# TechPizzaDev/VorbisPizza

Measured on AMD Instinct MI355X. Metric: decoded PCM Msamples/s (batched stereo N=2048), higher is better.
Workload: dtype f32; 1 GPU; north_star: batched stereo 44.1 kHz N=2048 IMDCT + window + overlap-add to PCM through the fused kernel (Mdct.Reverse + OverlapBuffers + StoreContiguous, Mdct.cs:15-19 + StreamDecoder.cs:764-791, 594-638): 65536 all-long frames x 2 ch per GPU (BASELINE configs[1]'s batch taken all the way to PCM), spectra N(0, 2^-8) device-resident, planar float32 PCM out, 8 B per sample; frames_per_gpu=65536, channels=2, block_size=2048, device_state=steady: 200 untimed steps of the workload in front of the W warm-up steps

## Files before the change

vorbispizza_amd/csrc/steady_stereo.hip:

```cpp
#include "imdct_core.hpp"
#include "steady_map.hpp"
#include "synth_common.hpp"
#include "synth_desc.hpp"
#include "vpz_internal.hpp"

namespace vpz {

constexpr int kSteadyWaves = 4;
constexpr int kSteadyThreads = 64 * kSteadyWaves;

__global__ __launch_bounds__(kSteadyThreads, 2) void steady_stereo_kernel(SynthArgs a)
{
    __shared__ float2 s_scr[kSteadyWaves][2][kWaveScratchFloat2];
    __shared__ int s_done[kSteadyWaves];

    const int lane = threadIdx.x & 63;
    const int wave = __builtin_amdgcn_readfirstlane(threadIdx.x >> 6);
    const int run_idx = (int)blockIdx.x * kSteadyWaves + wave;
    const bool active = run_idx < a.n_runs;
    RunDesc run = a.runs[active ? run_idx : 0];
    float2 rtw[8], rtwAB[8], rtwBC[8];
    float w_lo[8], w_hi[8];
    {
        const VPZ_GLOBAL float2 *tw = (const VPZ_GLOBAL float2 *)a.tw_long;
        const VPZ_GLOBAL float *sl = (const VPZ_GLOBAL float *)a.slope1;
#pragma unroll
        for (int m = 0; m < 8; ++m) {
            rtw[m] = tw[kFastTwOffset + lane + 64 * m];
            rtwAB[m] = tw[kFastTwABOffset + 64 * m + lane];
            rtwBC[m] = tw[kFastTwBCOffset + 8 * (lane & 7) + m];
            const int k = steady::cur_index(lane, m);
            w_lo[m] = sl[steady::sample_lo(k)];
            w_hi[m] = sl[steady::sample_hi(k)];
        }
    }
    if (threadIdx.x < kSteadyWaves) s_done[threadIdx.x] = 0;
    __syncthreads();
    if (!active) return;

    float2 *scrL = s_scr[wave][0], *scrR = s_scr[wave][1];
    const int n_staged = run.count + (run.pre_kind == kPreRecompute ? 1 : 0);
    const bool defer = run.pre_kind == kPreNeighbour && wave > 0 && run.count > 0;
    const bool first_emits = run.pre_kind == kPreState;
    const VPZ_GLOBAL float2 *src = (const VPZ_GLOBAL float2 *)(a.spec + run.spec_base);
    const VPZ_GLOBAL float2 *idle = (const VPZ_GLOBAL float2 *)a.inv_db;
    float *row_l, *row_r;
    {
        float *ob = a.out + (a.stream_out_off ? a.stream_out_off[run.stream] : 0) + run.out_base;
        const uint64_t p = reinterpret_cast<uint64_t>(ob);
        const uint32_t lo = __builtin_amdgcn_readfirstlane((uint32_t)p), hi = __builtin_amdgcn_readfirstlane((uint32_t)(p >> 32));
        row_l = reinterpret_cast<float *>(((uint64_t)hi << 32) | lo);
        row_r = row_l + a.channel_stride;
    }
    const bool clip_on = a.clip != 0;
    float clip_peak = 0.0f;

    float tL[8], tR[8];
#pragma unroll
    for (int q = 0; q < 8; ++q) tL[q] = tR[q] = 0.0f;
    if (run.pre_kind == kPreState) {
        const VPZ_GLOBAL float *st = (const VPZ_GLOBAL float *)(a.state_h + (size_t)run.state_slot * a.state_slot_floats + (size_t)run.stream * 2 * 1024);
#pragma unroll
        for (int q = 0; q < 8; ++q) {
            tL[q] = st[steady::tail_index(lane, q)];
            tR[q] = st[1024 + steady::tail_index(lane, q)];
        }
    }
    float parkL[8], parkR[8];
#pragma unroll
    for (int q = 0; q < 8; ++q) parkL[q] = parkR[q] = 0.0f;

    auto prefetch = [&](const VPZ_GLOBAL float2 *s2, bool valid, float2 (&va)[8], float2 (&vb)[8]) {
        int l = lane;
        asm volatile("" : "+v"(l));
        const VPZ_GLOBAL float2 *p = valid ? s2 : idle;
        const int base = valid ? l : 0, step = valid ? 64 : 0, rofs = valid ? 512 : 0;
#pragma unroll
        for (int m = 0; m < 8; ++m) {
            va[m] = p[base + step * m];
            vb[m] = p[base + step * m + rofs];
        }
    };
    auto emit = [&](const float (&curL)[8], const float (&curR)[8], const float (&pL)[8], const float (&pR)[8], float *out_l, float *out_r) {
        float loL[8], hiL[8], loR[8], hiR[8];
#pragma unroll
        for (int q = 0; q < 8; ++q) {
            loL[q] = ola(-curL[q], w_lo[q], pL[q], w_hi[q]);
            hiL[q] = ola(curL[q], w_hi[q], pL[q], w_lo[q]);
            loR[q] = ola(-curR[q], w_lo[q], pR[q], w_hi[q]);
            hiR[q] = ola(curR[q], w_hi[q], pR[q], w_lo[q]);
        }
        if (clip_on) {
#pragma unroll
            for (int q = 0; q < 8; q += 2) {
                clip_group(loL[q], hiL[q], loL[q + 1], hiL[q + 1], clip_peak);
                clip_group(loR[q], hiR[q], loR[q + 1], hiR[q + 1], clip_peak);
            }
        }
        int lf = lane;
        asm volatile("" : "+v"(lf));
#pragma unroll
        for (int q = 0; q < 8; ++q) {
            const float gotL = lane_mirror64(q < 4 ? hiL[7 - q] : loL[7 - q], lf);
            const float gotR = lane_mirror64(q < 4 ? hiR[7 - q] : loR[7 - q], lf);
            const int at = q < 4 ? 512 + 2 * (lf + 64 * q) : 2 * (lf + 64 * q) - 512;
            vpz_f2v vl = {q < 4 ? hiL[q] : loL[q], gotL}, vr = {q < 4 ? hiR[q] : loR[q], gotR};
            __builtin_nontemporal_store(vl, (VPZ_GLOBAL vpz_f2v *)reinterpret_cast<vpz_f2v *>(out_l + at));
            __builtin_nontemporal_store(vr, (VPZ_GLOBAL vpz_f2v *)reinterpret_cast<vpz_f2v *>(out_r + at));
        }
    };

    float2 va[8], vb[8];
    prefetch(src, n_staged > 0, va, vb);
#pragma unroll
    for (int m = 0; m < 8; ++m) asm volatile("" ::"v"(va[m].x), "v"(va[m].y), "v"(vb[m].x), "v"(vb[m].y));

    float *out_l = row_l + (defer ? 1024 : 0), *out_r = row_r + (defer ? 1024 : 0);
#ifdef VPZ_STAMPS
    unsigned long long t_acc[12] = {0, 0, 0, 0, 0, 0, 0, 0, 0, 0, 0, 0};
    unsigned long long t_last = __builtin_amdgcn_s_memtime();
#endif
    const int iters = n_staged;
    for (int it = 0; it < iters; ++it) {
        float2 na[8], nb[8];
        src += 1024;
        prefetch(src, it + 1 < iters, na, nb);
        VPZ_STAMP(0);
        int ln = lane;
        asm volatile("" : "+v"(ln));
        float reL[8], nimL[8], reR[8], nimR[8];
        imdct2048_wave_x2_spectrum(va, vb, scrL, scrR, rtw, rtwAB, rtwBC, ln, reL, nimL, reR, nimR);
        VPZ_STAMP(3);
#pragma unroll
        for (int m = 0; m < 8; ++m) asm volatile("" ::"v"(na[m].x), "v"(na[m].y), "v"(nb[m].x), "v"(nb[m].y));
        VPZ_STAMP(4);
        float curL[8], curR[8];
// ... 41 lines not shown
        float *pubL = reinterpret_cast<float *>(scrL), *pubR = reinterpret_cast<float *>(scrR);
#pragma unroll
        for (int q = 0; q < 8; ++q) {
            pubL[64 * q + lane] = tL[q];
            pubR[64 * q + lane] = tR[q];
        }
        __builtin_amdgcn_fence(__ATOMIC_RELEASE, "workgroup");
        if (lane == 0) __hip_atomic_store(&s_done[wave], 1, __ATOMIC_RELAXED, __HIP_MEMORY_SCOPE_WORKGROUP);
    }
    if (defer) {
        int spins = 0;
        while (__hip_atomic_load(&s_done[wave - 1], __ATOMIC_RELAXED, __HIP_MEMORY_SCOPE_WORKGROUP) == 0 && ++spins < (1 << 23))
            __builtin_amdgcn_s_sleep(4);
        __builtin_amdgcn_fence(__ATOMIC_ACQUIRE, "workgroup");
        const float *nbL = reinterpret_cast<const float *>(s_scr[wave - 1][0]), *nbR = reinterpret_cast<const float *>(s_scr[wave - 1][1]);
        float pL[8], pR[8];
#pragma unroll
        for (int q = 0; q < 8; ++q) {
            pL[q] = nbL[64 * q + lane];
            pR[q] = nbR[64 * q + lane];
        }
        emit(parkL, parkR, pL, pR, row_l, row_r);
    }
    if (run.flags & kRunSaveState) {
        VPZ_GLOBAL float *st = (VPZ_GLOBAL float *)(a.state_h + (size_t)(run.state_slot ^ 1) * a.state_slot_floats + (size_t)run.stream * 2 * 1024);
#pragma unroll
        for (int q = 0; q < 8; ++q) {
            st[steady::tail_index(lane, q)] = tL[q];
            st[1024 + steady::tail_index(lane, q)] = tR[q];
        }
    }
    if (clip_on && __any(clip_peak > 0.99999994f) && lane == 0) atomicMax(&a.clipped[run.stream], run.clip_epoch);
}

hipError_t launch_steady_stereo(const SynthArgs &args, hipStream_t stream)
{
    if (args.n_runs <= 0) return hipSuccess;
    if (args.channels != 2 || args.size0 != 256 || args.size1 != 2048 || args.interleaved || args.s16 || args.spec_i16 || args.ccount != nullptr)
        return hipErrorInvalidValue;
    const int grid = (args.n_runs + kSteadyWaves - 1) / kSteadyWaves;
    hipLaunchKernelGGL(steady_stereo_kernel, dim3(grid), dim3(kSteadyThreads), 0, stream, args);
    return hipGetLastError();
}

}
```

vorbispizza_amd/csrc/synth_plan.hip:

```cpp
#include <cstdio>
#include <cstdlib>
#include <cstring>

#include "synth_plan.hpp"

namespace vpz {

constexpr int kCutSkewPermille = 25;

namespace {

constexpr int64_t kNone = INT64_MAX;


struct Prev {
    bool has_prev, prev_long;
    int prev_end, prev_stop;
};
inline Prev prev_of_state(const StreamState &S) { return Prev{S.has_prev, S.prev_long, S.prev_end, S.prev_stop}; }
inline Prev prev_of(const Decoder &D, const vpz_packet *packets, int64_t p)
{
    if (p > 0 && packets[p - 1].stream == packets[p].stream) {
        const vpz_packet &pp = packets[p - 1];
        const PacketInfo &ppi = D.packet_info[pp.flags & 7];
// ... 709 lines not shown
        for (int g = s_lo; g < s_hi; ++g) {
            const int cnt = segs[g].cnt, base = (int)W.s_base[segs[g].stream] + segs[g].off;
            if (c.reuse) (void)code_segment<false>(P, c, segs[g]);
            int64_t before = 0, run_units = 0;
            for (int f0 = 0; f0 < cnt; before += run_units) {
                const int len = c.batches ? run_length(c, W.cut_code.data() + base, f0, cnt, target_at(P, c, g, before, c.target_units), run_units)
                                          : std::min(c.R + (c.skew_frames ? ((int64_t)base + f0 < c.heavy_frames ? 1 : -1) : 0), cnt - f0);
                const RunDesc r = make_run(P, segs[g], f0, len);
                if (c.parties > 1) mine.push_back(r);
                else if (P.n_runs < P.runs_cap) P.runs[P.n_runs++] = r;
                else { P.host_failed = true; return; }
                f0 += len;
            }
        }
    });
    if (c.parties == 1 || P.host_failed) return;
    for (const std::vector<RunDesc> &v : cut) {
        if (P.n_runs + v.size() > P.runs_cap) { P.host_failed = true; return; }
        memcpy(P.runs + P.n_runs, v.data(), v.size() * sizeof(RunDesc));
        P.n_runs += v.size();
    }
}

void chain_runs(SynthPlan &P)
{
    const Decoder &D = P.D;
    const vpz_packet *packets = P.packets;
    RunDesc *runs = P.runs;
    const size_t n_runs = P.n_runs;
    P.n_chained = 0;
    if (!P.use_dual || !P.compact || D.size1 != 2048 || D.no_chain) return;
    const size_t waves = (size_t)P.dual_waves;
    auto chain_range = [&](size_t lo, size_t hi) -> int64_t {
        int64_t n = 0;
        for (size_t i = std::max<size_t>(lo, 1); i < hi; ++i) {
            RunDesc &r = runs[i];
            const RunDesc &pr = runs[i - 1];
            if (i % waves == 0 || r.pre_kind != kPreRecompute || r.stream != pr.stream || pr.count <= 0 ||
                r.first != pr.first + pr.count || !(r.flags & kRunCompact) || r.count <= 0)
                continue;
            const int64_t q = r.first;
            if (q <= 0 || packets[q - 1].stream != r.stream) continue;
            const uint8_t cf = P.cflags[q], pcf = P.cflags[q - 1];
            if ((cf & (7u | kCfSkip)) != 7u || (pcf & (1u | 4u | kCfSkip)) != 5u) continue;
            if (r.count == 1 && (r.flags & kRunLastTrimmed)) continue;
            r.pre_kind = kPreNeighbour;
            stage_from(P, r, q);
            ++n;
        }
        return n;
    };
    const bool want_inline = P.cut_R > 0 && P.cut_R + 1 <= 16;
    P.run_inline = want_inline ? arena_alloc<uint8_t>(*P.A, 32 * n_runs + 32) : nullptr;
    auto inline_range = [&](size_t lo, size_t hi) {
        for (size_t i = lo; want_inline && i < hi; ++i) {
            const RunDesc &r = runs[i];
            uint8_t *dst = P.run_inline + 32 * i;
            memset(dst, 0, 32);
            if (!(r.flags & kRunCompact)) continue;
            const int64_t q = (int64_t)r.first + (r.pre_kind == kPreRecompute ? -1 : 0);
            const int n = std::min(16, r.count + (r.pre_kind == kPreRecompute ? 1 : 0));
            for (int j = 0; j < n; ++j) {
                dst[j] = P.cflags[q + j];
                dst[16 + j] = P.cmap[q + j];
            }
        }
    };
    P.chain_threads = 1;
    if (P.pool && P.pool->parties() > 1 && n_runs >= 1024) {
        const int n_threads = P.chain_threads = P.pool->parties();
        std::vector<int64_t> part((size_t)n_threads, 0);
        P.host_failed |= !P.pool->run([&](int party) {
            const size_t lo = n_runs * (size_t)party / n_threads, hi = n_runs * (size_t)(party + 1) / n_threads;
            part[(size_t)party] = chain_range(lo, hi);
            inline_range(lo, hi);
        });
        for (int64_t v : part) P.n_chained += v;
    } else {
        P.n_chained = chain_range(0, n_runs);
        inline_range(0, n_runs);
    }
}

bool all_steady(const SynthPlan &P, const Cut &c)
{
    const Decoder &D = P.D;
    if (!P.use_dual || D.pairs || !P.compact || c.batches || D.no_steady || D.channels != 2 || D.size0 != 256 || D.size1 != 2048) return false;
    if (!P.facts.all_steady_flags || P.facts.any_floor || P.facts.any_short || P.facts.ilv_seen || !D.mismatch_packets.empty()) return false;
    for (int s = 0; s < D.n_streams; ++s) {
        if (D.plan.s_cnt[s] <= 0) continue;
        const StreamState &S = D.states[s];
        if (S.has_prev && !(S.prev_long && S.prev_end == 1024 && S.prev_stop == 2048)) return false;
        if (D.plan.trim_out_count[s] >= 0) return false;
    }
    return true;
}

}

bool SynthPlan::dual_usable() const
{
    if (!D.dual_ok || (facts.any_floor0 && !D.f0_fused) || (facts.ilv_seen && facts.planar_seen)) return false;
    const bool wide = facts.ilv_seen && !D.pairs;
// ... 38 lines not shown
                  W.cut_hint_R > 0;
        if (c.batches && W.cut_code.size() < (size_t)total_frames) W.cut_code.resize((size_t)total_frames);
        if (c.batches) W.s_units.assign((size_t)n_segs, 0);
        c.total_units = (c.batches && !c.reuse) ? count_units(P, c) : 8 * total_frames;
        c.R = W.cut_hint_R;
        c.run_slots = W.cut_hint_slots;
        c.single_round = false;
        if (!c.reuse) choose_run_length(P, c);
        c.min_run_frames = std::max(1, c.R - 1 - (c.R >= 16 ? c.R * kCutSkewPermille / 1000 + 2 : 0));
        P.runs_cap = (size_t)(total_frames / c.min_run_frames) + (size_t)std::max(n_segs, D.n_streams) + 1;
        P.runs = arena_alloc<RunDesc>(*P.A, P.runs_cap);
        if (D.generic) return;
        fit_target(P, c);
        if (!c.batches && !c.skew_frames && P.pool && P.pool->parties() > 1 && total_frames / std::max(1, c.R) >= 1024)
            write_runs_by_length_wide(P, c);
        else
            write_runs_per_segment(P, c);
        if (P.host_failed) { P.n_runs = 0; return; }
        if (!(c.reuse && ((int64_t)P.n_runs > c.run_slots || (int64_t)P.n_runs * 10 < W.cut_hint_runs * 9))) break;
        W.cut_hint_frames = -1;
    }
    if (c.batches && !c.reuse) W.cut_hint_runs = (int64_t)P.n_runs;
    P.cut_R = c.R;
    chain_runs(P);
    P.steady = all_steady(P, c);
    if (getenv("VPZ_HOST_PROFILE"))
        fprintf(stderr, "[vpz host] cut: %s, by %s, R %d, target %lld eighths, %zu runs for %lld slots, %d segments on %d threads, heavy below %lld, "
                        "hint (frames %lld, runs %lld), chained %lld, runs filled by %s on %d threads, chain sweep on %d threads\n",
                c.reuse ? "hint reused" : "fitted", c.batches ? "cost" : "length", c.R,
                (long long)c.target_units, P.n_runs, (long long)c.run_slots, n_segs, c.parties, (long long)c.heavy_work,
                (long long)W.cut_hint_frames, (long long)W.cut_hint_runs, (long long)P.n_chained,
                P.fill_threads > 1 ? "the pool" : "the calling thread", P.fill_threads, P.chain_threads);
}

}
```

vorbispizza_amd/csrc/synth_plan.hpp:

```cpp
#pragma once

#include <algorithm>

#include "host_pool.hpp"
#include "vpz_decoder.hpp"

namespace vpz {

struct BatchFacts {
    bool any_floor = false, any_floor0 = false, need_coupling = false;
    bool any_short = false;
    bool ilv_seen = false, planar_seen = false;
    bool group_align_ok = true;
    bool align2_ok = true;
    bool all_steady_flags = true;
    int64_t res_extent = 0;
    void note(const Decoder &D, const vpz_packet &pk)
    {
        const bool bf = pk.flags & VPZ_PKT_BLOCK_FLAG;
        if (!bf) any_short = true;
        res_extent = std::max(res_extent, pk.residue_offset + (int64_t)D.channels * ((bf ? D.size1 : D.size0) / 2));
        if (!(pk.flags & VPZ_PKT_NO_FLOOR)) {
            any_floor = true;
            if (D.mappings[pk.mapping].coupling_steps > 0) need_coupling = true;
            if (D.mapping_uses_floor0[pk.mapping]) any_floor0 = true;
        }
        if (pk.flags & VPZ_PKT_INTERLEAVED) { need_coupling = true; ilv_seen = true; }
// ... 24 lines not shown
    HostPool *pool = nullptr;
    int parties = 1;
    int dual_waves = 1;
    bool needs_general = false;
    int64_t (*resident_slots)(const SynthPlan &) = nullptr;
    std::vector<StreamState> st;
    std::vector<uint8_t> started_with_prev, started_prev_long;
    FrameDesc *frames = nullptr;
    size_t n_frames = 0;
    uint8_t *rec_floor = nullptr;
    BatchFacts facts;
    bool was_parallel = false;
    bool use_group = false;
    bool use_dual = false;
    bool cut_by_cost = false;
    bool compact = false;
    uint8_t *cflags = nullptr, *cmap = nullptr;
    uint8_t *run_inline = nullptr;
    RunDesc *runs = nullptr;
    size_t n_runs = 0, runs_cap = 0;
    bool host_failed = false;
    int64_t n_chained = 0;
    bool steady = false;
    int cut_R = 0;
    int fill_threads = 1, chain_threads = 1;

    int64_t capacity_of(int s) const
    {
        return D.stream_caps.empty() ? stream_out_capacity : std::min(stream_out_capacity, D.stream_caps[(size_t)s]);
    }
    bool dual_usable() const;
    bool group_usable() const;
};

int plan_frames(SynthPlan &P, int64_t *samples_written);
void plan_runs(SynthPlan &P);

}
```

vorbispizza_amd/csrc/vpz_decoder.hip:

```cpp
#include <algorithm>
#include <chrono>
#include <cstdio>
#include <cstdlib>
#include <cstring>
#include <new>
#include <vector>

#include "synth_plan.hpp"
#include "../../include/vorbispizza_synth_debug.h"

namespace vpz {

static const uint32_t k_inverse_db_bits[256] = {
#include "floor1_inverse_db_bits.inc"
};

constexpr size_t kZeroCopyMax = 8u << 20;
__global__ __launch_bounds__(256) void widen_i16_kernel(const int16_t *__restrict__ in, float *__restrict__ out, long n)
{
    const long stride = (long)gridDim.x * 256 * 8;
    if ((reinterpret_cast<uintptr_t>(in) & 15) == 0) {
        for (long i = ((long)blockIdx.x * 256 + threadIdx.x) * 8; i < n; i += stride) {
            if (i + 8 <= n) {
                const uint4 v = *reinterpret_cast<const uint4 *>(in + i);
// ... 140 lines not shown
    D.size1 = cfg->block_size1;
    D.clip = cfg->clip_samples ? 1 : 0;
    D.n_streams = n_streams;
    {
        const char *no_big = getenv("VPZ_NO_BIG");
        D.big = synth_big_supported(cfg->block_size0, cfg->block_size1) && !(no_big && atoi(no_big));
    }
    D.generic = !synth_supports_sizes(cfg->block_size0, cfg->block_size1) && !D.big;
    D.states.assign(n_streams, StreamState());
    D.floors.assign((size_t)cfg->floor_count, vpz_floor1_config{});
    D.floor_types.assign((size_t)cfg->floor_count, 1);
    D.floors0.assign((size_t)cfg->floor_count, vpz_floor0_config{});
    for (int i = 0; i < cfg->floor_count; ++i) {
        if (cfg->floor_types) D.floor_types[i] = cfg->floor_types[i];
        if (D.floor_types[i] == 1 && cfg->floors) D.floors[i] = cfg->floors[i];
        if (D.floor_types[i] == 0 && cfg->floors0) D.floors0[i] = cfg->floors0[i];
    }
    D.mappings.assign(cfg->mappings, cfg->mappings + cfg->mapping_count);
    static_assert(VPZ_PKT_BLOCK_FLAG == 1 && VPZ_PKT_PREV_FLAG == 2 && VPZ_PKT_NEXT_FLAG == 4, "packet_info index");
    for (int f = 0; f < 8; ++f) D.packet_info[f] = get_packet_info(D.size0, D.size1, f & 1, f & 2, f & 4);
    if (const char *e = getenv("VPZ_NO_DIRECT_I16")) D.no_direct_i16 = atoi(e) != 0;
    if (const char *e = getenv("VPZ_NO_CHAIN")) D.no_chain = atoi(e) != 0;
    if (const char *e = getenv("VPZ_NO_STEADY")) D.no_steady = atoi(e) != 0;
    if (const char *e = getenv("VPZ_DUAL_RUN")) D.dual_run = std::max(4, atoi(e));
    if (const char *e = getenv("VPZ_PLAN_SLOTS")) D.plan_slots = std::max<int64_t>(0, atoll(e));
    if (const char *e = getenv("VPZ_SYNTH_ABLATE")) D.ablate = atoi(e);
    if (const char *e = getenv("VPZ_HOST_THREADS")) D.host_threads = atoi(e);
    if (const char *e = getenv("VPZ_NO_EARLY_UPLOAD")) D.no_early_upload = atoi(e) != 0;
    if (const char *e = getenv("VPZ_PAR_MIN_PACKETS")) D.par_min_packets = atoll(e);

    int rc = VPZ_OK;
    std::vector<FloorDev> fdev(std::max<size_t>(1, D.floors.size()));
    for (size_t i = 0; i < D.floors.size() && rc == VPZ_OK; ++i) {
        if (D.floor_types[i] == 1) {
            rc = build_floor(D.floors[i], &fdev[i]);
        } else if (D.floor_types[i] == 0) {
            const vpz_floor0_config &f0 = D.floors0[i];
            if (f0.order < 1 || f0.order > 255 || f0.rate < 1 || f0.bark_map_size < 1 || f0.amp_bits < 0 || f0.amp_bits > 63)
                rc = VPZ_E_INVALID_ARG;
        } else {
            rc = VPZ_E_INVALID_ARG;
        }
    }
    std::vector<uint8_t> steps;
    for (size_t m = 0; m < D.mappings.size() && rc == VPZ_OK; ++m) {
        const vpz_mapping_config &mc = D.mappings[m];
// ... 348 lines not shown
    int64_t early_res_extent = 0;

    SynthCall(Decoder &dec, int64_t n, const vpz_packet *pk, const float *res, const int16_t *po, const uint8_t *pc,
              int mem, void *out, const int64_t *out_off, int64_t out_cap, int layout, int64_t stride)
        : D(dec), ctx(dec.ctx), n_packets(n), packets(pk), residue(res), posts(po), post_counts(pc), mem_space(mem),
          pcm_out(out), stream_out_offset(out_off), stream_out_capacity(out_cap), out_layout(layout),
          channel_stride(stride), C(dec.channels), half0(dec.size0 / 2), half1(dec.size1 / 2),
          n_rec(n * dec.channels), have_posts(po && pc && !dec.floors.empty()),
          out_interleaved(layout == VPZ_OUT_INTERLEAVED || layout == VPZ_OUT_INTERLEAVED_S16),
          out_s16(layout == VPZ_OUT_INTERLEAVED_S16 || layout == VPZ_OUT_PLANAR_S16),
          out_elem(out_s16 ? sizeof(int16_t) : sizeof(float)),
          P{dec, n, pk, have_posts, mem, reinterpret_cast<uintptr_t>(res), out_interleaved, out_cap}
    {
    }

    void *dev(const void *host_ptr) const
    {
        if (!host_ptr) return nullptr;
        char *base = zero_copy ? A->mapped : static_cast<char *>(A->dev.p);
        return base + (static_cast<const char *>(host_ptr) - A->base);
    }
    bool zero_copy = false;
    bool steady_kernel = false;

    int resolved_parties = 0;
    int host_parties()
    {
        if (resolved_parties > 0) return resolved_parties;
        int parties = D.host_threads;
        if (parties <= 0) {
            cpu_set_t set;
            parties = sched_getaffinity(0, sizeof set, &set) == 0 ? CPU_COUNT(&set) : (int)std::thread::hardware_concurrency();
            if (const char *lw = getenv("LOCAL_WORLD_SIZE")) parties /= std::max(1, atoi(lw));
            parties = std::max(1, std::min(parties, 16));
        }
        return resolved_parties = parties;
    }
    HostPool *own_pool()
    {
        const int parties = host_parties();
        HostPool *pool = static_cast<HostPool *>(ctx->host_pool);
        if (n_packets >= D.par_min_packets && parties >= 2 && !(pool && pool->parties() == parties)) {
            if (pool) ctx->host_pool_free(pool);
            ctx->host_pool = pool = new HostPool(parties);
            ctx->host_pool_free = [](void *p) { delete static_cast<HostPool *>(p); };
        }
        return pool && parties >= 2 && pool->parties() == parties ? pool : nullptr;
// ... 409 lines not shown
        a.channel_stride = dev_channel_stride;
        a.interleaved = out_interleaved;
        a.s16 = out_s16 ? 1 : 0;
        a.clip = D.clip;
        a.clipped = D.d_clipped;
        a.no_batch = ((D.ablate & 128) || !P.cut_by_cost || P.facts.any_floor0) ? 1 : 0;
        a.ablate = D.ablate;
        a.stamps = nullptr;
#if defined(VPZ_STAMPS) || defined(VPZ_WAVE_TIMES)
        static unsigned long long *d_stamps = nullptr;
        constexpr size_t kStampWaves = 1 << 16;
        if (!d_stamps) (void)hipMalloc(&d_stamps, (16 + 16 * kStampWaves) * sizeof(unsigned long long));
        (void)hipMemsetAsync(d_stamps, 0, (16 + 16 * std::min<size_t>(kStampWaves, P.n_runs)) * sizeof(unsigned long long), ctx->stream);
        a.stamps = d_stamps;
#endif
        steady_kernel = false;
        if (P.steady && !out_interleaved && !out_s16 && !spec_i16) {
            int64_t bits = (int64_t)reinterpret_cast<uintptr_t>(d_out) / (int64_t)sizeof(float) | dev_channel_stride;
            if (reinterpret_cast<uintptr_t>(d_out) % sizeof(float)) bits |= 1;
            for (int s = 0; s < D.n_streams; ++s)
                if (D.plan.s_cnt[s] > 0) bits |= offs[s];
            steady_kernel = (bits & 1) == 0;
        }
        hipError_t e = steady_kernel ? launch_steady_stereo(a, ctx->stream)
                     : P.use_dual ? (D.pairs ? launch_synth_pairs(a, P.facts.any_floor, P.facts.ilv_seen, ctx->stream) : launch_synth_dual(a, P.facts.any_floor, P.facts.ilv_seen, ctx->stream))
                                : D.big ? launch_synth_big(a, P.facts.any_floor, ctx->stream) : launch_synth(a, P.facts.any_floor, ctx->stream);
        if (e != hipSuccess) return set_error(ctx, VPZ_E_HIP, "synth kernel launch", e);
#if defined(VPZ_STAMPS) || defined(VPZ_WAVE_TIMES)
        {
            unsigned long long h[16];
            (void)hipMemcpyAsync(h, d_stamps, sizeof(h), hipMemcpyDeviceToHost, ctx->stream);
            (void)hipStreamSynchronize(ctx->stream);
            static const char *names_one[9] = {"desc+prefetch", "barrier0", "stage+barrier", "coupling", "pickup+curve",
                                               "floor*+imdct", "wait next", "ola+stores", "tail"};
            static const char *names_dual[9] = {"desc+prefetch", "unpack+coupling", "curves", "floor*+imdct x2", "wait next",
                                                "ola+stores", "tail", "-", "-"};
            const char **names = P.use_dual ? names_dual : names_one;
            unsigned long long tot = 0;
            for (int k = 0; k < 9; ++k) tot += h[k];
            fprintf(stderr, "[stamps] %llu waves, %.0f cycles per wave:", h[15], h[15] ? (double)tot / h[15] : 0.0);
            for (int k = 0; k < 9; ++k) fprintf(stderr, " %s %.1f%%", names[k], tot ? 100.0 * h[k] / tot : 0.0);
            if (h[14] && h[15]) {
                const double mean = (double)tot / h[15], var = (double)h[13] * 1e6 / h[15] - mean * mean;
                fprintf(stderr, " | slowest wave %.0f cycles = %.2f x mean, sigma %.2f x mean, %.1f passes per wave, %d runs", (double)h[14],
                        (double)h[14] / mean, var > 0 ? sqrt(var) / mean : 0.0, (double)h[12] / h[15], (int)P.n_runs);
            }
            fprintf(stderr, "\n");
// ... 85 lines not shown
        }
    } early_guard{ctx, call};
    if (!D.no_early_upload && (rc = call.stage_inputs_early(residue_floats, n_records)) != VPZ_OK) return rc;
    if ((rc = call.open_arena()) != VPZ_OK) return rc;
    const auto t_arena = tick();
    if ((rc = call.plan_frames(samples_written)) != VPZ_OK) return rc;
    const SynthPlan &plan = call.P;
    if (plan.facts.res_extent > residue_floats)
        return set_error(ctx, VPZ_E_INVALID_ARG, "vpz_decoder_synth: a packet's residue lies beyond residue_floats");
    const auto t_pass1 = tick();
    if (plan.n_frames == 0) {
        D.states = plan.st;
        return VPZ_OK;
    }
    plan_runs(call.P);
    if (plan.host_failed) return set_error(ctx, VPZ_E_NOMEM, "vpz_decoder_synth: run cutting failed (allocation)");
    call.build_coupling_packets();
    if ((rc = call.build_floor0_records()) != VPZ_OK) return rc;
    if ((rc = call.build_output_offsets()) != VPZ_OK) return rc;
    call.build_generic_lists();
    const auto t_pass2 = tick();
    if ((rc = call.stage_inputs()) != VPZ_OK) return rc;
    if ((rc = call.launch()) != VPZ_OK) return rc;
    if (call.zero_copy) {
        VPZ_HIP_TRY(ctx, hipEventRecord(call.A->uploaded, ctx->stream));
        call.A->pending = true;
    }
    if ((rc = call.copy_back()) != VPZ_OK) return rc;
    early_guard.completed = mem_space == VPZ_MEM_HOST;
    if (!D.generic)
        for (int s = 0; s < D.n_streams; ++s)
            if (D.plan.s_cnt[s] > 0) call.P.st[s].state_slot ^= 1;
    D.states = plan.st;
    if (host_profile) {
        const auto t_end = tick();
        auto us = [](auto a, auto b) { return std::chrono::duration<double, std::micro>(b - a).count(); };
        const char *route = D.generic ? "generic" : plan.use_dual ? (D.pairs ? "pairs" : "stereo") : D.big ? "big" : plan.use_group ? "group" : "separate";
        fprintf(stderr, "[vpz host] packets %lld: route %s, kernel %s, arena wait %.1f us, pass1 %.1f us (%s), runs %.1f us, uploads+launch %.1f us\n",
                (long long)n_packets, route, call.steady_kernel ? "steady" : "general", us(t_begin, t_arena), us(t_arena, t_pass1), plan.was_parallel ? "parallel" : "serial",
                us(t_pass1, t_pass2), us(t_pass2, t_end));
    }
    return VPZ_OK;
}

int vpz_decoder_synth(vpz_decoder *d, int64_t n_packets, const vpz_packet *packets, const float *residue,
                      int64_t residue_floats, const int16_t *posts, const uint8_t *post_counts, int64_t n_records,
                      int mem_space, void *pcm_out, const int64_t *stream_out_offset, int64_t stream_out_capacity,
                      int out_layout, int64_t channel_stride, int64_t *samples_written)
{
    if (!d) return VPZ_E_INVALID_ARG;
    try {
        return synth_impl(d, n_packets, packets, residue, residue_floats, posts, post_counts, n_records, mem_space, pcm_out,
                          stream_out_offset, stream_out_capacity, out_layout, channel_stride, samples_written);
    } catch (const ArenaOverflow &) {
        return set_error(d->impl.ctx, VPZ_E_NOMEM, "vpz_decoder_synth: the descriptor arena is too small for this batch");
    } catch (const std::bad_alloc &) {
        return set_error(d->impl.ctx, VPZ_E_NOMEM, "vpz_decoder_synth: host allocation failed");
    } catch (...) {
        return set_error(d->impl.ctx, VPZ_E_NOMEM, "vpz_decoder_synth: host pass failed");
    }
}

int vpz_decoder_last_packet_status(vpz_decoder *d, int32_t *out, int64_t capacity, int64_t *n_not_ok)
// ... 161 lines not shown
```

vorbispizza_amd/csrc/vpz_decoder.hpp:

```cpp
#pragma once

#include <vector>

#include "vpz_internal.hpp"

namespace vpz {

struct StreamState {
    bool has_prev = false;
    bool prev_long = false;
    int prev_start = 0, prev_end = 0, prev_stop = 0;
    int64_t current_position = 0;
    bool has_position = true;
    bool eos_found = false;
    bool has_clipped = false;
    int32_t clip_epoch = 1;
    int32_t state_slot = 0;
};

using DevBuf = Scratch;

struct PinnedArena {
    char *base = nullptr;
    char *mapped = nullptr;
// ... 74 lines not shown
    DevBuf b_ybuf;
    DevBuf b_bigtail;
    bool generic = false;
    bool big = false;
    std::vector<uint8_t> floor_types;
    std::vector<vpz_floor0_config> floors0;
    void *d_floors0 = nullptr;
    int32_t *d_bark_maps = nullptr;
    bool f0_fused = false;
    bool has_floor1 = false;
    int f0_k = 0;
    uint16_t *d_f0_bark = nullptr;
    float *d_f0_w = nullptr;
    DevBuf b_f0curve;
    DevBuf b_in_amp, b_in_coeff;
    const float *f0_amp = nullptr, *f0_coeff = nullptr;
    int32_t f0_stride = 0;
    PacketInfo packet_info[8];
    int dual_run = 8;
    int64_t plan_slots = 0;
    bool no_direct_i16 = false;
    bool no_chain = false;
    bool no_steady = false;
    int ablate = 0;
    bool no_early_upload = false;
    std::vector<int32_t> packet_samples;
    std::vector<int64_t> mismatch_packets;
};

}
```

vorbispizza_amd/csrc/vpz_internal.hpp:

```cpp
#pragma once

#include <hip/hip_runtime.h>

#include <array>
#include <cstdint>
#include <map>
#include <string>
#include <utility>
#include <vector>

#include "../../include/vorbispizza_synth.h"
#include "../../include/vorbispizza_pcm_pack.h"
#include "synth_desc.hpp"

namespace vpz {

struct BlockTables {
    int n = 0;
    float2 *d_fast = nullptr;
    float *d_A = nullptr, *d_B = nullptr, *d_C = nullptr;
    uint16_t *d_bitrev = nullptr;
    int ld = 0;
    float *d_slope = nullptr;
    std::vector<float> h_slope;
};

struct Context;

struct Scratch {
    void *p = nullptr;
    size_t bytes = 0;
    bool drain = false;
    int grow(Context *ctx, size_t need, const char *what);
};

// ... 107 lines not shown
                              const uint16_t *bitrev, int num_cu, hipStream_t stream,
                              const int64_t *src_off = nullptr, const int64_t *dst_off = nullptr);

hipError_t launch_floor1_unwrap(int n_rec, const int16_t *posts, const uint8_t *post_counts, const uint8_t *rec_info,
                                const FloorDev *floors, int n_floors, int32_t *cposts, uint8_t *ccount, int16_t *dbg_y,
                                uint8_t *dbg_f, hipStream_t stream, int f0_fused = 0);
hipError_t launch_floor0_curves(int n_rec, const uint8_t *rec_info, const void *floors, const float *amp, const float *coeff,
                                int coeff_stride, int k_stride, const float *wtab, float *curve, const uint8_t *post_counts,
                                uint8_t *ccount, int32_t *cposts, hipStream_t stream);
hipError_t launch_floor0_wtab(const void *floors, int n_floors, int k_stride, float *wtab, hipStream_t stream);
hipError_t launch_floor1_render(int n_rec, const int32_t *cposts, const uint8_t *ccount, const uint8_t *rec_info,
                                int half0, int half1, uint8_t *curve_y, hipStream_t stream);
hipError_t launch_coupling(const void *pkts, int n_pkts, const uint8_t *steps, int channels,
                           const float *residue, float *temp, int max_half, hipStream_t stream);
hipError_t launch_synth(const SynthArgs &args, bool has_floor, hipStream_t stream);
bool synth_supports_sizes(int size0, int size1);
bool synth_needs_general(int size0, int size1);
int synth_resident_waves(bool has_floor, int num_cu, int channels, bool group);
bool synth_group_supported(int channels);
bool synth_dual_supported(int channels, int size0, int size1);
hipError_t launch_synth_dual(const SynthArgs &args, bool has_floor, bool interleaved_in, hipStream_t stream);
int synth_dual_resident_slots(bool has_floor, int num_cu);
int synth_dual_waves();
hipError_t launch_steady_stereo(const SynthArgs &args, hipStream_t stream);
bool synth_pairs_supported(int channels, int size0, int size1);
hipError_t launch_synth_pairs(const SynthArgs &args, bool has_floor, bool interleaved_in, hipStream_t stream);
bool synth_big_supported(int size0, int size1);
hipError_t launch_synth_big(const SynthArgs &args, bool has_floor, hipStream_t stream);
int synth_big_resident_waves(bool has_floor, int num_cu, int size0, int size1);
int64_t synth_big_tail_floats(int size1, int64_t n_items);
hipError_t launch_generic_floor(const GenericFrame *frames, int n_frames, int channels, int half1, float *spec,
                                const uint8_t *post_counts, const uint8_t *curve_y, const float *inv_db,
                                hipStream_t stream);
hipError_t launch_generic_ola(const GenericFrame *frames, int n_frames, int channels, int size0, int size1,
                              const float *ybuf, float *state_y, const float *slope0, const float *slope1, float *out,
                              const int64_t *stream_out_off, int64_t channel_stride, int interleaved, int clip,
                              int32_t *clipped, int s16, hipStream_t stream);
hipError_t launch_generic_save_state(const GenericFrame *frames, const int32_t *save_list, int n_save, int channels,
                                     int size1, const float *ybuf, float *state_y, hipStream_t stream);
hipError_t launch_floor0_apply(const void *recs, int n_recs, const void *floors, const int32_t *bark_maps,
                               const float *amp, const float *coeff, int coeff_stride, float *spec,
                               hipStream_t stream);
size_t floor0_dev_size();
size_t floor0_rec_size();
void fill_floor0_dev(void *dst, int order, int bark_map_size, int amp_ofs, int64_t off_short, int64_t off_long);
void fill_floor0_rec(void *dst, int64_t spec_off, int rec, int floor, int half, int is_long);
size_t coupling_packet_size();
// ... 19 lines not shown
```

Baseline: 665,700 Msamples/s.

## Derive steady run descriptors on device from a segment table in kernel args

Each wave now computes its run descriptor from a small segment table passed by value in the kernel argument block, using a binary search. This replaces reading a per-run RunDesc array from the uploaded arena, which also lets the spectrum prefetch be issued before the twiddle and window loads. The host checks that the derived descriptors match the host-built ones before enabling the path. When nothing else reads the arena, it skips the arena-upload event record. Costs: a larger argument block, extra host verification work, and a per-wave binary search.

New measurement: 665,700 Msamples/s. Within noise of the previous version (-0.0%).

```diff
diff --git a/vorbispizza_amd/csrc/steady_runs.hpp b/vorbispizza_amd/csrc/steady_runs.hpp
--- /dev/null
+++ b/vorbispizza_amd/csrc/steady_runs.hpp
@@ -0,0 +1,88 @@
+#pragma once
+
+#include <cstdint>
+
+#if defined(__HIPCC__)
+#define VPZ_STEADY_HD __host__ __device__
+#else
+#define VPZ_STEADY_HD
+#endif
+
+namespace vpz {
+
+constexpr int kSteadyMaxSegs = 64;
+
+namespace steady {
+constexpr int32_t kRunPreNone = 0, kRunPreState = 1, kRunPreRecompute = 2, kRunPreNeighbour = 3;
+constexpr int kFrameFloats = 2 * 1024;
+constexpr int kFrameSamples = 1024;
+}
+
+struct SteadySeg {
+    int64_t spec_base;
+    int64_t out_base;
+    int32_t first_run;
+    int32_t frames;
+    int32_t frames_before;
+    int32_t stream;
+    int32_t clip_epoch;
+    uint8_t from_state;
+    uint8_t ends_stream;
+    uint8_t state_slot;
+    uint8_t pad;
+};
+static_assert(sizeof(SteadySeg) == 40, "SteadySeg layout");
+
+struct SteadyRun {
+    int32_t count, stream, pre_kind;
+    int64_t spec_base, out_base;
+    bool save_state;
+    int32_t state_slot, clip_epoch;
+};
+
+VPZ_STEADY_HD inline int64_t steady_emitting(const SteadySeg &g, int64_t p)
+{
+    return g.from_state ? p : (p > 0 ? p - 1 : 0);
+}
+
+VPZ_STEADY_HD inline SteadyRun steady_run(const SteadySeg *segs, int n_segs, int R, int waves, bool chain_on, int run_idx)
+{
+    int lo = 0, hi = n_segs - 1;
+    while (lo < hi) {
+        const int mid = (lo + hi + 1) >> 1;
+        if (segs[mid].first_run <= run_idx) lo = mid;
+        else hi = mid - 1;
+    }
+    const SteadySeg &g = segs[lo];
+    const int k = run_idx - g.first_run;
+    const int64_t f0 = (int64_t)k * R;
+    const int64_t p = g.frames_before + f0;
+    const int64_t left = g.frames - f0;
+    SteadyRun r;
+    r.count = (int32_t)(left < R ? left : R);
+    r.stream = g.stream;
+    r.state_slot = g.state_slot;
+    r.clip_epoch = g.clip_epoch;
+    r.save_state = g.ends_stream && f0 + r.count >= g.frames;
+    r.out_base = g.out_base + (steady_emitting(g, p) - steady_emitting(g, g.frames_before)) * steady::kFrameSamples;
+    int64_t staged = f0;
+    if (p == 0) {
+        r.pre_kind = g.from_state ? steady::kRunPreState : steady::kRunPreNone;
+    } else {
+        bool same_stream = k > 0;
+        if (!same_stream && lo > 0) {
+            const SteadySeg &b = segs[lo - 1];
+            same_stream = b.stream == g.stream && b.frames_before + b.frames == g.frames_before;
+        }
+        if (chain_on && run_idx % waves != 0 && same_stream) {
+            r.pre_kind = steady::kRunPreNeighbour;
+        } else {
+            r.pre_kind = steady::kRunPreRecompute;
+            staged = f0 - 1;
+        }
+    }
+    r.spec_base = g.spec_base + staged * steady::kFrameFloats;
+    return r;
+}
+
+}
diff --git a/vorbispizza_amd/csrc/steady_stereo.hip b/vorbispizza_amd/csrc/steady_stereo.hip
--- a/vorbispizza_amd/csrc/steady_stereo.hip
+++ b/vorbispizza_amd/csrc/steady_stereo.hip
@@ -1,5 +1,6 @@
 #include "imdct_core.hpp"
 #include "steady_map.hpp"
+#include "steady_runs.hpp"
 #include "synth_common.hpp"
 #include "synth_desc.hpp"
 #include "vpz_internal.hpp"
@@ -9,7 +10,34 @@
 constexpr int kSteadyWaves = 4;
 constexpr int kSteadyThreads = 64 * kSteadyWaves;
 
-__global__ __launch_bounds__(kSteadyThreads, 2) void steady_stereo_kernel(SynthArgs a)
+static_assert(steady::kRunPreNone == kPreNone && steady::kRunPreState == kPreState && steady::kRunPreRecompute == kPreRecompute &&
+                  steady::kRunPreNeighbour == kPreNeighbour,
+              "steady_runs.hpp names the pre kinds of synth_desc.hpp");
+
+struct SteadyArgs {
+    const float *spec;
+    const float *inv_db;
+    float *state_h;
+    int64_t state_slot_floats;
+    const float2 *tw_long;
+    const float *slope1;
+    float *out;
+    int64_t channel_stride;
+    int32_t *clipped;
+    unsigned long long *stamps;
+    const RunDesc *runs;
+    const int64_t *stream_out_off;
+    int32_t clip;
+    int32_t n_runs;
+    int32_t R;
+    int32_t chain_on;
+    int32_t n_segs;
+    SteadySeg segs[kSteadyMaxSegs];
+};
+static_assert(sizeof(SteadyArgs) <= 3072, "the argument block stays well inside the 4 KiB a launch may pass");
+
+template <bool kDeviceRuns>
+__global__ __launch_bounds__(kSteadyThreads, 2) void steady_stereo_kernel(SteadyArgs a)
 {
     __shared__ float2 s_scr[kSteadyWaves][2][kWaveScratchFloat2];
     __shared__ int s_done[kSteadyWaves];
@@ -18,7 +46,36 @@
     const int wave = __builtin_amdgcn_readfirstlane(threadIdx.x >> 6);
     const int run_idx = (int)blockIdx.x * kSteadyWaves + wave;
     const bool active = run_idx < a.n_runs;
-    RunDesc run = a.runs[active ? run_idx : 0];
+    SteadyRun run;
+    if constexpr (kDeviceRuns) {
+        run = steady_run(a.segs, a.n_segs, a.R, kSteadyWaves, a.chain_on != 0, active ? run_idx : 0);
+    } else {
+        const RunDesc rd = a.runs[active ? run_idx : 0];
+        run.count = rd.count;
+        run.stream = rd.stream;
+        run.pre_kind = rd.pre_kind;
+        run.spec_base = rd.spec_base;
+        run.out_base = rd.out_base;
+        run.save_state = (rd.flags & kRunSaveState) != 0;
+        run.state_slot = rd.state_slot;
+        run.clip_epoch = rd.clip_epoch;
+    }
+    const int n_staged = run.count + (run.pre_kind == kPreRecompute ? 1 : 0);
+    const VPZ_GLOBAL float2 *src = (const VPZ_GLOBAL float2 *)(a.spec + run.spec_base);
+    const VPZ_GLOBAL float2 *idle = (const VPZ_GLOBAL float2 *)a.inv_db;
+    auto prefetch = [&](const VPZ_GLOBAL float2 *s2, bool valid, float2 (&va)[8], float2 (&vb)[8]) {
+        int l = lane;
+        asm volatile("" : "+v"(l));
+        const VPZ_GLOBAL float2 *p = valid ? s2 : idle;
+        const int base = valid ? l : 0, step = valid ? 64 : 0, rofs = valid ? 512 : 0;
+#pragma unroll
+        for (int m = 0; m < 8; ++m) {
+            va[m] = p[base + step * m];
+            vb[m] = p[base + step * m + rofs];
+        }
+    };
+    float2 va[8], vb[8];
+    if constexpr (kDeviceRuns) prefetch(src, active && n_staged > 0, va, vb);
     float2 rtw[8], rtwAB[8], rtwBC[8];
     float w_lo[8], w_hi[8];
     {
@@ -39,14 +96,12 @@
     if (!active) return;
 
     float2 *scrL = s_scr[wave][0], *scrR = s_scr[wave][1];
-    const int n_staged = run.count + (run.pre_kind == kPreRecompute ? 1 : 0);
     const bool defer = run.pre_kind == kPreNeighbour && wave > 0 && run.count > 0;
     const bool first_emits = run.pre_kind == kPreState;
-    const VPZ_GLOBAL float2 *src = (const VPZ_GLOBAL float2 *)(a.spec + run.spec_base);
-    const VPZ_GLOBAL float2 *idle = (const VPZ_GLOBAL float2 *)a.inv_db;
     float *row_l, *row_r;
     {
-        float *ob = a.out + (a.stream_out_off ? a.stream_out_off[run.stream] : 0) + run.out_base;
+        float *ob = a.out + run.out_base;
+        if constexpr (!kDeviceRuns) ob += a.stream_out_off ? a.stream_out_off[run.stream] : 0;
         const uint64_t p = reinterpret_cast<uint64_t>(ob);
         const uint32_t lo = __builtin_amdgcn_readfirstlane((uint32_t)p), hi = __builtin_amdgcn_readfirstlane((uint32_t)(p >> 32));
         row_l = reinterpret_cast<float *>(((uint64_t)hi << 32) | lo);
@@ -70,17 +125,6 @@
 #pragma unroll
     for (int q = 0; q < 8; ++q) parkL[q] = parkR[q] = 0.0f;
 
-    auto prefetch = [&](const VPZ_GLOBAL float2 *s2, bool valid, float2 (&va)[8], float2 (&vb)[8]) {
-        int l = lane;
-        asm volatile("" : "+v"(l));
-        const VPZ_GLOBAL float2 *p = valid ? s2 : idle;
-        const int base = valid ? l : 0, step = valid ? 64 : 0, rofs = valid ? 512 : 0;
-#pragma unroll
-        for (int m = 0; m < 8; ++m) {
-            va[m] = p[base + step * m];
-            vb[m] = p[base + step * m + rofs];
-        }
-    };
     auto emit = [&](const float (&curL)[8], const float (&curR)[8], const float (&pL)[8], const float (&pR)[8], float *out_l, float *out_r) {
         float loL[8], hiL[8], loR[8], hiR[8];
 #pragma unroll
@@ -110,8 +154,7 @@
         }
     };
 
-    float2 va[8], vb[8];
-    prefetch(src, n_staged > 0, va, vb);
+    if constexpr (!kDeviceRuns) prefetch(src, n_staged > 0, va, vb);
 #pragma unroll
     for (int m = 0; m < 8; ++m) asm volatile("" ::"v"(va[m].x), "v"(va[m].y), "v"(vb[m].x), "v"(vb[m].y));
 
@@ -199,7 +242,7 @@
         }
         emit(parkL, parkR, pL, pR, row_l, row_r);
     }
-    if (run.flags & kRunSaveState) {
+    if (run.save_state) {
         VPZ_GLOBAL float *st = (VPZ_GLOBAL float *)(a.state_h + (size_t)(run.state_slot ^ 1) * a.state_slot_floats + (size_t)run.stream * 2 * 1024);
 #pragma unroll
         for (int q = 0; q < 8; ++q) {
@@ -210,13 +253,37 @@
     if (clip_on && __any(clip_peak > 0.99999994f) && lane == 0) atomicMax(&a.clipped[run.stream], run.clip_epoch);
 }
 
-hipError_t launch_steady_stereo(const SynthArgs &args, hipStream_t stream)
+hipError_t launch_steady_stereo(const SynthArgs &args, const SteadySeg *segs, int n_segs, int R, bool chain_on, hipStream_t stream)
 {
     if (args.n_runs <= 0) return hipSuccess;
     if (args.channels != 2 || args.size0 != 256 || args.size1 != 2048 || args.interleaved || args.s16 || args.spec_i16 || args.ccount != nullptr)
         return hipErrorInvalidValue;
+    if (segs && (n_segs < 1 || n_segs > kSteadyMaxSegs || R < 1)) return hipErrorInvalidValue;
+    SteadyArgs a{};
+    a.spec = args.spec;
+    a.inv_db = args.inv_db;
+    a.state_h = args.state_h;
+    a.state_slot_floats = args.state_slot_floats;
+    a.tw_long = args.tw_long;
+    a.slope1 = args.slope1;
+    a.out = args.out;
+    a.channel_stride = args.channel_stride;
+    a.clipped = args.clipped;
+    a.stamps = args.stamps;
+    a.clip = args.clip;
+    a.n_runs = args.n_runs;
     const int grid = (args.n_runs + kSteadyWaves - 1) / kSteadyWaves;
-    hipLaunchKernelGGL(steady_stereo_kernel, dim3(grid), dim3(kSteadyThreads), 0, stream, args);
+    if (segs) {
+        a.R = R;
+        a.chain_on = chain_on ? 1 : 0;
+        a.n_segs = n_segs;
+        for (int g = 0; g < n_segs; ++g) a.segs[g] = segs[g];
+        hipLaunchKernelGGL(steady_stereo_kernel<true>, dim3(grid), dim3(kSteadyThreads), 0, stream, a);
+    } else {
+        a.runs = args.runs;
+        a.stream_out_off = args.stream_out_off;
+        hipLaunchKernelGGL(steady_stereo_kernel<false>, dim3(grid), dim3(kSteadyThreads), 0, stream, a);
+    }
     return hipGetLastError();
 }
 
diff --git a/vorbispizza_amd/csrc/synth_plan.hip b/vorbispizza_amd/csrc/synth_plan.hip
--- a/vorbispizza_amd/csrc/synth_plan.hip
+++ b/vorbispizza_amd/csrc/synth_plan.hip
@@ -755,6 +755,39 @@
     }
 }
 
+bool steady_table(SynthPlan &P)
+{
+    const Decoder &D = P.D;
+    const PlanScratch &W = D.plan;
+    P.n_steady_segs = 0;
+    P.device_runs = false;
+    if (!P.steady || D.no_device_runs || P.mem_space != VPZ_MEM_DEVICE || P.cut_R < 1) return false;
+    int n = 0;
+    int64_t first_run = 0;
+    for (const CutSeg &seg : W.cut_segs) {
+        if (seg.cnt <= 0) continue;
+        if (n == kSteadyMaxSegs) return false;
+        const int s = seg.stream;
+        const int64_t q = W.s_base[s] + seg.off;
+        SteadySeg &g = P.steady_segs[n++];
+        g = SteadySeg{};
+        g.spec_base = P.packets[q].residue_offset;
+        g.out_base = W.out_off_scratch[(size_t)q];
+        g.first_run = (int32_t)first_run;
+        g.frames = seg.cnt;
+        g.frames_before = seg.off;
+        g.stream = s;
+        g.clip_epoch = D.states[s].clip_epoch;
+        g.from_state = P.started_with_prev[s] ? 1 : 0;
+        g.ends_stream = seg.off + seg.cnt >= (int)W.s_cnt[s] ? 1 : 0;
+        g.state_slot = (uint8_t)D.states[s].state_slot;
+        first_run += (seg.cnt + P.cut_R - 1) / P.cut_R;
+    }
+    if (n == 0 || first_run != (int64_t)P.n_runs) return false;
+    P.n_steady_segs = n;
+    return true;
+}
+
 void chain_runs(SynthPlan &P)
 {
     const Decoder &D = P.D;
@@ -762,8 +795,23 @@
     RunDesc *runs = P.runs;
     const size_t n_runs = P.n_runs;
     P.n_chained = 0;
-    if (!P.use_dual || !P.compact || D.size1 != 2048 || D.no_chain) return;
     const size_t waves = (size_t)P.dual_waves;
+    const bool prove = steady_table(P);
+    auto derived_range = [&](size_t lo, size_t hi) -> bool {
+        for (size_t i = lo; i < hi; ++i) {
+            const SteadyRun d = steady_run(P.steady_segs, P.n_steady_segs, P.cut_R, (int)waves, !D.no_chain, (int)i);
+            const RunDesc &r = runs[i];
+            if (d.count != r.count || d.stream != r.stream || d.pre_kind != r.pre_kind || d.spec_base != r.spec_base ||
+                d.out_base != r.out_base || d.save_state != ((r.flags & kRunSaveState) != 0) || d.state_slot != r.state_slot ||
+                d.clip_epoch != r.clip_epoch)
+                return false;
+        }
+        return true;
+    };
+    if (!P.use_dual || !P.compact || D.size1 != 2048 || D.no_chain) {
+        if (prove) P.device_runs = derived_range(0, n_runs);
+        return;
+    }
     auto chain_range = [&](size_t lo, size_t hi) -> int64_t {
         int64_t n = 0;
         for (size_t i = std::max<size_t>(lo, 1); i < hi; ++i) {
@@ -803,15 +851,20 @@
     if (P.pool && P.pool->parties() > 1 && n_runs >= 1024) {
         const int n_threads = P.chain_threads = P.pool->parties();
         std::vector<int64_t> part((size_t)n_threads, 0);
+        std::vector<uint8_t> derived((size_t)n_threads, 0);
         P.host_failed |= !P.pool->run([&](int party) {
             const size_t lo = n_runs * (size_t)party / n_threads, hi = n_runs * (size_t)(party + 1) / n_threads;
             part[(size_t)party] = chain_range(lo, hi);
             inline_range(lo, hi);
+            derived[(size_t)party] = prove && derived_range(lo, hi);
         });
         for (int64_t v : part) P.n_chained += v;
+        P.device_runs = prove && !P.host_failed;
+        for (uint8_t ok : derived) P.device_runs = P.device_runs && ok;
     } else {
         P.n_chained = chain_range(0, n_runs);
         inline_range(0, n_runs);
+        P.device_runs = prove && derived_range(0, n_runs);
     }
 }
 
@@ -896,8 +949,8 @@
     }
     if (c.batches && !c.reuse) W.cut_hint_runs = (int64_t)P.n_runs;
     P.cut_R = c.R;
+    P.steady = all_steady(P, c);
     chain_runs(P);
-    P.steady = all_steady(P, c);
     if (getenv("VPZ_HOST_PROFILE"))
         fprintf(stderr, "[vpz host] cut: %s, by %s, R %d, target %lld eighths, %zu runs for %lld slots, %d segments on %d threads, heavy below %lld, "
                         "hint (frames %lld, runs %lld), chained %lld, runs filled by %s on %d threads, chain sweep on %d threads\n",
diff --git a/vorbispizza_amd/csrc/synth_plan.hpp b/vorbispizza_amd/csrc/synth_plan.hpp
--- a/vorbispizza_amd/csrc/synth_plan.hpp
+++ b/vorbispizza_amd/csrc/synth_plan.hpp
@@ -3,6 +3,7 @@
 #include <algorithm>
 
 #include "host_pool.hpp"
+#include "steady_runs.hpp"
 #include "vpz_decoder.hpp"
 
 namespace vpz {
@@ -73,6 +74,9 @@
     bool host_failed = false;
     int64_t n_chained = 0;
     bool steady = false;
+    SteadySeg steady_segs[kSteadyMaxSegs];
+    int n_steady_segs = 0;
+    bool device_runs = false;
     int cut_R = 0;
     int fill_threads = 1, chain_threads = 1;
 
diff --git a/vorbispizza_amd/csrc/vpz_decoder.hip b/vorbispizza_amd/csrc/vpz_decoder.hip
--- a/vorbispizza_amd/csrc/vpz_decoder.hip
+++ b/vorbispizza_amd/csrc/vpz_decoder.hip
@@ -186,6 +186,8 @@
     if (const char *e = getenv("VPZ_NO_DIRECT_I16")) D.no_direct_i16 = atoi(e) != 0;
     if (const char *e = getenv("VPZ_NO_CHAIN")) D.no_chain = atoi(e) != 0;
     if (const char *e = getenv("VPZ_NO_STEADY")) D.no_steady = atoi(e) != 0;
+    if (const char *e = getenv("VPZ_NO_DEVICE_RUNS")) D.no_device_runs = atoi(e) != 0;
+    if (const char *e = getenv("VPZ_ARENA_EVENT")) D.keep_arena_event = atoi(e) != 0;
     if (const char *e = getenv("VPZ_DUAL_RUN")) D.dual_run = std::max(4, atoi(e));
     if (const char *e = getenv("VPZ_PLAN_SLOTS")) D.plan_slots = std::max<int64_t>(0, atoll(e));
     if (const char *e = getenv("VPZ_SYNTH_ABLATE")) D.ablate = atoi(e);
@@ -580,7 +582,7 @@
     }
     bool zero_copy = false;
     bool steady_kernel = false;
-
+    bool device_runs = false;
     int resolved_parties = 0;
     int host_parties()
     {
@@ -1036,7 +1038,13 @@
                 if (D.plan.s_cnt[s] > 0) bits |= offs[s];
             steady_kernel = (bits & 1) == 0;
         }
-        hipError_t e = steady_kernel ? launch_steady_stereo(a, ctx->stream)
+        device_runs = steady_kernel && P.device_runs && mem_space == VPZ_MEM_DEVICE;
+        SteadySeg segs[kSteadyMaxSegs];
+        for (int g = 0; device_runs && g < P.n_steady_segs; ++g) {
+            segs[g] = P.steady_segs[g];
+            segs[g].out_base += offs[segs[g].stream];
+        }
+        hipError_t e = steady_kernel ? launch_steady_stereo(a, device_runs ? segs : nullptr, P.n_steady_segs, P.cut_R, !D.no_chain, ctx->stream)
                      : P.use_dual ? (D.pairs ? launch_synth_pairs(a, P.facts.any_floor, P.facts.ilv_seen, ctx->stream) : launch_synth_dual(a, P.facts.any_floor, P.facts.ilv_seen, ctx->stream))
                                 : D.big ? launch_synth_big(a, P.facts.any_floor, ctx->stream) : launch_synth(a, P.facts.any_floor, ctx->stream);
         if (e != hipSuccess) return set_error(ctx, VPZ_E_HIP, "synth kernel launch", e);
@@ -1168,7 +1176,9 @@
     const auto t_pass2 = tick();
     if ((rc = call.stage_inputs()) != VPZ_OK) return rc;
     if ((rc = call.launch()) != VPZ_OK) return rc;
-    if (call.zero_copy) {
+    const bool others_read_arena = plan.facts.any_floor || plan.facts.any_floor0 || D.generic ||
+                                   (plan.facts.need_coupling && !plan.use_group && !plan.use_dual);
+    if (call.zero_copy && (!call.device_runs || others_read_arena || D.keep_arena_event)) {
         VPZ_HIP_TRY(ctx, hipEventRecord(call.A->uploaded, ctx->stream));
         call.A->pending = true;
     }
@@ -1182,9 +1192,9 @@
         const auto t_end = tick();
         auto us = [](auto a, auto b) { return std::chrono::duration<double, std::micro>(b - a).count(); };
         const char *route = D.generic ? "generic" : plan.use_dual ? (D.pairs ? "pairs" : "stereo") : D.big ? "big" : plan.use_group ? "group" : "separate";
-        fprintf(stderr, "[vpz host] packets %lld: route %s, kernel %s, arena wait %.1f us, pass1 %.1f us (%s), runs %.1f us, uploads+launch %.1f us\n",
+        fprintf(stderr, "[vpz host] packets %lld: route %s, kernel %s, arena wait %.1f us, pass1 %.1f us (%s), runs %.1f us, uploads+launch %.1f us, runs %s\n",
                 (long long)n_packets, route, call.steady_kernel ? "steady" : "general", us(t_begin, t_arena), us(t_arena, t_pass1), plan.was_parallel ? "parallel" : "serial",
-                us(t_pass1, t_pass2), us(t_pass2, t_end));
+                us(t_pass1, t_pass2), us(t_pass2, t_end), call.device_runs ? "device" : "arena");
     }
     return VPZ_OK;
 }
diff --git a/vorbispizza_amd/csrc/vpz_decoder.hpp b/vorbispizza_amd/csrc/vpz_decoder.hpp
--- a/vorbispizza_amd/csrc/vpz_decoder.hpp
+++ b/vorbispizza_amd/csrc/vpz_decoder.hpp
@@ -120,6 +120,8 @@
     bool no_direct_i16 = false;
     bool no_chain = false;
     bool no_steady = false;
+    bool no_device_runs = false;
+    bool keep_arena_event = false;
     int ablate = 0;
     bool no_early_upload = false;
     std::vector<int32_t> packet_samples;
diff --git a/vorbispizza_amd/csrc/vpz_internal.hpp b/vorbispizza_amd/csrc/vpz_internal.hpp
--- a/vorbispizza_amd/csrc/vpz_internal.hpp
+++ b/vorbispizza_amd/csrc/vpz_internal.hpp
@@ -11,6 +11,7 @@
 
 #include "../../include/vorbispizza_synth.h"
 #include "../../include/vorbispizza_pcm_pack.h"
+#include "steady_runs.hpp"
 #include "synth_desc.hpp"
 
 namespace vpz {
@@ -164,7 +165,7 @@
 hipError_t launch_synth_dual(const SynthArgs &args, bool has_floor, bool interleaved_in, hipStream_t stream);
 int synth_dual_resident_slots(bool has_floor, int num_cu);
 int synth_dual_waves();
-hipError_t launch_steady_stereo(const SynthArgs &args, hipStream_t stream);
+hipError_t launch_steady_stereo(const SynthArgs &args, const SteadySeg *segs, int n_segs, int R, bool chain_on, hipStream_t stream);
 bool synth_pairs_supported(int channels, int size0, int size1);
 hipError_t launch_synth_pairs(const SynthArgs &args, bool has_floor, bool interleaved_in, hipStream_t stream);
 bool synth_big_supported(int size0, int size1);
```
